# zjwzcx/GenNBV

Measured on AMD Instinct MI355X. Metric: env-steps/sec at 256 envs x 64^3 grid (state encoding + policy forward + GAE + PPO update), higher is better.
Workload: dtype f32

## Files before the change

gennbv_amd/csrc/conv_split.h:

```cpp
#pragma once
#include <type_traits>

typedef _Float16 h8 __attribute__((ext_vector_type(8)));
typedef _Float16 h4 __attribute__((ext_vector_type(4)));
typedef _Float16 h2 __attribute__((ext_vector_type(2)));

namespace split {
constexpr int kThreads = 1024, kWaves = 16;
constexpr int kConsWaves = 8, kProdThreads = 512;
constexpr int kNP = 4, kNPl = 2 * kNP + 1;
constexpr int kRing = 5;
constexpr int kRowBytes = 2048;
constexpr int kStageBytes = kNPl * kRing * kRowBytes;
constexpr int kPadBytes = 64;
constexpr int kSlots = (2 * kNPl * 128 + kProdThreads - 1) / kProdThreads;
constexpr int kRedBytes = 2 * kNP * 1024;
constexpr int kDyBytes = 2 * kNP * 1024;
constexpr int kGradBits = 14;
constexpr int kLdsBytes = kStageBytes + kPadBytes + kRedBytes;
constexpr int kWgLdsBytes = kStageBytes + kPadBytes + kDyBytes;
constexpr int kKSteps = 14, kKHalf = 7;
constexpr float kZScale = 256.0f, kWScale = 1024.0f, kZMax = 65000.0f;
constexpr int kW2ImgU4 = kKSteps * 2 * 64;

// ... 411 lines not shown
constexpr int kChunks = 5;
static_assert(4 * split::kNPl + split::kNP == kChunks * (split::kWaves - split::kConsWaves), "40 chunks over 8 staging waves");
}

__device__ __forceinline__ void glds16_nt(const void *gsrc, uint32_t lds_dst)
{
    uint32_t keep;
    asm volatile("s_mov_b32 %0, m0\n\ts_mov_b32 m0, %2\n\ts_nop 0\n\tglobal_load_lds_dwordx4 %1, off nt\n\ts_mov_b32 m0, %0"
                 : "=&s"(keep) : "v"(gsrc), "s"(lds_dst) : "memory");
}
template <int N>
__device__ __forceinline__ void wait_vm_keep()
{
    asm volatile("s_waitcnt vmcnt(%0)" ::"n"(N) : "memory");
}
__device__ __forceinline__ uint32_t lds_addr(const void *p)
{
    return (uint32_t)(uintptr_t)(__attribute__((address_space(3))) const char *)p;
}

__global__ __launch_bounds__(split::kThreads) void k_conv2_wgrad_split_dma(
    const float *__restrict__ y1, const float *__restrict__ scale1, const float *__restrict__ shift1, const float *__restrict__ dy2 ,
    const unsigned *__restrict__ absmax, int B, int O1, int O2, int nitems, float *__restrict__ partial )
{
    using namespace split;
    extern __shared__ __attribute__((aligned(16))) char split_lds[];
    char *stage = split_lds, *dyst = split_lds + wdma::kStageBytes + kPadBytes;
    constexpr int R = wdma::kRing;
    const int tid = threadIdx.x, lane = tid & (kWave - 1), wv = __builtin_amdgcn_readfirstlane(tid / kWave);
    constexpr int E2 = kTaps * 256 + kC;
    float *out = partial + (size_t)blockIdx.x * E2;
    if (tid < kPadBytes / 16) reinterpret_cast<uint4 *>(split_lds + wdma::kStageBytes)[tid] = make_uint4(0, 0, 0, 0);
    const int P2 = O2 * O2 * O2;
    const int nsteps = (O2 + 1) & ~1;
    if (wv >= kConsWaves) {
        const int pw = wv - kConsWaves, q = lane & 3, vx = lane >> 2;
        const bool dy_wave = pw >= 4;
        const uint32_t rowC = 2 * 16 * kC, planeC = rowC * (uint32_t)O1;
        const int dpl = pw - 4;
        const uint32_t stage_a = lds_addr(stage), dy_a = lds_addr(dyst);
        float gs = 1.0f, sc[4] = {0.f, 0.f, 0.f, 0.f}, sh[4] = {0.f, 0.f, 0.f, 0.f};
        bool first = true;
        for (int item = (int)blockIdx.x; item < nitems; item += (int)gridDim.x) {
            int b, oz0, oz1;
            if (!sample_plane_group(B, O2, kNP, b, oz0, oz1, item)) continue;
            const int np = oz1 - oz0, npl = 2 * np + 1;
            const float *ybase = y1 + ((size_t)b * O1 + 2 * oz0) * planeC + lane * 4;
            const bool dvalid = dy_wave && dpl < np && vx < O2;
            const float *dsrc = dy2 + ((size_t)b * P2 + (size_t)(oz0 + min(max(dpl, 0), np - 1)) * O2 * O2 + min(vx, O2 - 1)) * kC + 4 * q;
            auto issue = [&](int j) {
#ifdef WDMA_ABL_NODMA
                return;
#endif
#pragma unroll
                for (int k = 0; k < wdma::kChunks; ++k) {
                    if (k == wdma::kChunks - 1 && dy_wave) {
                        glds16_nt(dsrc + (size_t)min(max(j, 0), O2 - 1) * O2 * kC, __builtin_amdgcn_readfirstlane(dy_a + (uint32_t)((((j + 3) % wdma::kDyBufs) * kNP + dpl) * 1024)));
                    } else {
                        const int h = pw + 8 * k, pi = h >> 2, row = 2 * j + 1 + ((h >> 1) & 1), slot = (row + 2 * R) % R;
                        const float *src = ybase + (uint32_t)min(pi, npl - 1) * planeC + (uint32_t)min(max(row, 0), O1 - 1) * rowC + (h & 1) * (16 * kC);
                        glds16_nt(src, __builtin_amdgcn_readfirstlane(stage_a + (uint32_t)((pi * R + slot) * kRowBytes + (h & 1) * 1024)));
                    }
                }
            };
            auto convert = [&](int j) {
#ifdef WDMA_ABL_NOCONV
                return;
#endif
                char *cp[wdma::kChunks];
                float4 raw[wdma::kChunks];
#pragma unroll
                for (int k = 0; k < wdma::kChunks; ++k) {
                    if (k == wdma::kChunks - 1 && dy_wave) {
                        cp[k] = dyst + (((j + 3) % wdma::kDyBufs) * kNP + dpl) * 1024;
                    } else {
                        const int h = pw + 8 * k, pi = h >> 2, row = 2 * j + 1 + ((h >> 1) & 1), slot = (row + 2 * R) % R;
                        cp[k] = stage + (pi * R + slot) * kRowBytes + (h & 1) * 1024;
                    }
                    raw[k] = *reinterpret_cast<const float4 *>(cp[k] + lane * 16);
                }
#pragma unroll
                for (int k = 0; k < wdma::kChunks; ++k) {
                    float z[4];
                    const float v[4] = {raw[k].x, raw[k].y, raw[k].z, raw[k].w};
                    if (k == wdma::kChunks - 1 && dy_wave) {
#pragma unroll
                        for (int e = 0; e < 4; ++e) z[e] = dvalid ? v[e] * gs : 0.0f;
                    } else {
                        const bool pad_voxel = ((pw + 8 * k) & 1) == 1 && vx == 15;
#pragma unroll
                        for (int e = 0; e < 4; ++e) z[e] = pad_voxel ? 0.0f : __builtin_amdgcn_fmed3f(fmaf(sc[e], v[e], sh[e]), 0.f, kZMax);
                    }
                    h4 hi, lo;
#pragma unroll
                    for (int e = 0; e < 4; ++e) {
                        _Float16 a, c2;
                        split2(z[e], a, c2);
                        hi[e] = a;
                        lo[e] = c2;
                    }
                    char *dst = cp[k] + vx * 32 + q * 8;
                    *reinterpret_cast<h4 *>(dst) = hi;
#ifndef SPLIT_HI_ONLY
                    *reinterpret_cast<h4 *>(dst + 512) = lo;
#endif
                }
            };
            issue(-1);
            issue(0);
            if (first) {
                gs = grad_scale(absmax);
#pragma unroll
                for (int s = 0; s < 4; ++s) {
                    sc[s] = scale1[4 * q + s] * kZScale;
                    sh[s] = shift1[4 * q + s] * kZScale;
                }
                first = false;
            }
#pragma unroll
            for (int s = 0; s < 4; ++s) asm volatile("" : "+v"(sc[s]), "+v"(sh[s]));
            wait_vm_keep<0>();
            convert(-1);
            issue(1);
            convert(0);
            split_step_barrier();
            for (int t = 1; t <= nsteps; ++t) {
                issue(t + 1);
                wait_vm_keep<wdma::kChunks>();
                convert(t);
                split_step_barrier();
            }
            wait_vm_keep<0>();
        }
    } else {
        const float gs = grad_scale(absmax);
        const int n = lane & 15, g = lane >> 4, cw = wv;
        const int ntaps = cw < 3 ? 4 : 3;
        uint32_t tapbase[4];
        int tapdy[4];
#pragma unroll
        for (int i = 0; i < 4; ++i) {
            const int tp = min(cw + 8 * i, kTaps - 1), dz = tp / 9, dy = (tp / 3) % 3, dx = tp % 3;
            tapbase[i] = (uint32_t)(dz * R * kRowBytes + (dx == 1 ? 1024 : 0) + (dx == 2 ? 32 : 0)) + lane * 8;
            tapdy[i] = dy;
        }
        f32x4 acc[4];
#pragma unroll
        for (int i = 0; i < 4; ++i) acc[i] = (f32x4){0.f, 0.f, 0.f, 0.f};
        h8 ones;
#pragma unroll
        for (int e = 0; e < 8; ++e) ones[e] = (_Float16)1.0f;
        for (int item = (int)blockIdx.x; item < nitems; item += (int)gridDim.x) {
            int b, oz0, oz1;
            if (!sample_plane_group(B, O2, kNP, b, oz0, oz1, item)) continue;
            const int np = oz1 - oz0;
            split_step_barrier();
            for (int t = 1; t <= nsteps; ++t) {
                const int oy = t - 1;
#ifdef WDMA_ABL_NOCOMP
                if (false) {
#else
                if (oy < O2) {
#endif
                    uint32_t rowoff[3];
#pragma unroll
                    for (int dy = 0; dy < 3; ++dy) rowoff[dy] = (uint32_t)(((2 * oy + dy) % R) * kRowBytes);
                    const char *dybuf = dyst + (oy % wdma::kDyBufs) * kNP * 1024 + lane * 8;
#pragma unroll
                    for (int kb = 0; kb < 2; ++kb) {
                        if (2 * kb < np) {
                            const h8 bh = tr_pair(dybuf + (2 * kb) * 1024, dybuf + (2 * kb + 1) * 1024);
                            const h8 bl = tr_pair(dybuf + (2 * kb) * 1024 + 512, dybuf + (2 * kb + 1) * 1024 + 512);
                            h8 ah[4], al[4];
#pragma unroll
                            for (int i = 0; i < 4; ++i) {
                                if (i < 3 || ntaps == 4) {
                                    const uint32_t off = tapbase[i] + (tapdy[i] == 0 ? rowoff[0] : tapdy[i] == 1 ? rowoff[1] : rowoff[2]);
                                    const char *a0 = stage + (2 * (2 * kb)) * R * kRowBytes + off, *a1 = a0 + 2 * R * kRowBytes;
                                    ah[i] = tr_pair(a0, a1);
                                    al[i] = tr_pair(a0 + 512, a1 + 512);
                                }
                            }
#pragma unroll
                            for (int i = 0; i < 3; ++i) acc[i] = mfma_h(ah[i], bh, acc[i]);
                            if (ntaps == 4) acc[3] = mfma_h(ah[3], bh, acc[3]);
#pragma unroll
                            for (int i = 0; i < 3; ++i) acc[i] = mfma_lo(al[i], bh, acc[i]);
                            if (ntaps == 4) acc[3] = mfma_lo(al[3], bh, acc[3]);
#pragma unroll
                            for (int i = 0; i < 3; ++i) acc[i] = mfma_lo(ah[i], bl, acc[i]);
                            if (ntaps == 4) acc[3] = mfma_lo(ah[3], bl, acc[3]);
                            if (cw == 7) {
                                acc[3] = mfma_h(ones, bh, acc[3]);
                                acc[3] = mfma_lo(ones, bl, acc[3]);
                            }
                        }
                    }
                }
                split_step_barrier();
            }
// ... 465 lines not shown
    const float *__restrict__ dy2, const uint4 *__restrict__ w2img , const float *__restrict__ wbound ,
    const unsigned *__restrict__ absmax, const float *__restrict__ y1,
    const float *__restrict__ scale1, const float *__restrict__ shift1, const float *__restrict__ mean1, const float *__restrict__ rstd1,
    const int8_t *__restrict__ grid_i8, const int64_t *__restrict__ rows, int64_t grid_row_stride, int B, int G, int O1, int O2,
    float *__restrict__ partial )
{
    conv2_dgrad_c1w_split_body(dy2, w2img, wbound, absmax, y1, scale1, shift1, mean1, rstd1, grid_i8, rows, grid_row_stride, B, G, O1, O2, partial,
                               (int)blockIdx.x);
}


namespace fsplit {
constexpr int kInPlanes = 2 * split::kNPl + 1;
constexpr int kInRows = 5;
constexpr int kInRowBytes = 128, kInPlaneBytes = kInRows * kInRowBytes;
constexpr int kInBuf = kInPlanes * kInPlaneBytes + 64;
constexpr int kInPieces = kInPlanes * kInRows * 4;
constexpr int kTilesPerStep = 2 * split::kNPl * 2;
constexpr int kCompWaves = 4, kStageWaves = 12;
constexpr int kTilesPerWave = kTilesPerStep / kStageWaves;
static_assert(kTilesPerWave * kStageWaves == kTilesPerStep && kStageWaves % 4 == 0 && (kCompWaves + kStageWaves) * 64 == split::kThreads, "tile split");
constexpr float kW1Scale = 1024.0f;
constexpr int kLdsBytes = split::kStageBytes + split::kPadBytes + split::kRedBytes + 2 * kInBuf;
}

__global__ void k_prep_w2_split_only(const float *__restrict__ W2, float *__restrict__ w2img)
{
    prep_w2_split_items<true>(W2, w2img, blockIdx.x * blockDim.x + threadIdx.x, gridDim.x * blockDim.x);
}

template <bool TRAIN>
__global__ __launch_bounds__(split::kThreads) void k_conv12_fwd_split(
    const int8_t *__restrict__ grid_i8, const int64_t *__restrict__ rows, int64_t grid_row_stride, const float *__restrict__ W1 ,
    const float *__restrict__ b1, const float *__restrict__ scale1, const float *__restrict__ shift1, int B, int G, int O1, int O2,
    const uint4 *__restrict__ w2img, const float *__restrict__ b2, float *__restrict__ y2, float *__restrict__ y1 ,
    float *__restrict__ partials )
{
    using namespace split;
    using namespace fsplit;
    extern __shared__ __attribute__((aligned(16))) char split_lds[];
    char *stage = split_lds;
    float *red = reinterpret_cast<float *>(split_lds + split::kStageBytes + kPadBytes);
    char *inbuf = split_lds + split::kStageBytes + kPadBytes + kRedBytes;
    int b, oz0, oz1;
    const bool live = sample_plane_group(B, O2, kNP, b, oz0, oz1);
    const int tid = threadIdx.x, lane = tid & (kWave - 1), wv = __builtin_amdgcn_readfirstlane(tid / kWave);
    if (!live) {
        if (TRAIN) write_partials(partials, kWaves, wv, 0.f, 0.f);
        return;
    }
    const int np = oz1 - oz0;
    const int nsteps = (O2 + 2) & ~1;
    float s_sum = 0.0f, s_sq = 0.0f;
    if (wv >= kCompWaves) {
        const int ptid = tid - kCompWaves * kWave, pw = min(max(wv - kCompWaves, 0), kStageWaves - 1);
        const int n = lane & 15, g = lane >> 4;
        h8 wh, wl, wh2, wl2;
#pragma unroll
        for (int e = 0; e < 8; ++e) {
            const int r = 2 * g + (e >> 2), dx = e & 3;
            _Float16 hi, lo;
            split2(dx < 3 ? W1[n * kTaps + 3 * r + dx] * kW1Scale : 0.0f, hi, lo);
            wh[e] = hi;
            wl[e] = lo;
            split2(g == 0 && e < 3 ? W1[n * kTaps + 24 + e] * kW1Scale : 0.0f, hi, lo);
            wh2[e] = hi;
            wl2[e] = lo;
        }
        const int rsel = (pw >> 1) & 1, par = pw & 1;
        auto row_addr = [&](int r) {
            return (uint32_t)(split::kStageBytes + kPadBytes + kRedBytes + (r / 3 + 2 * (pw >> 2)) * kInPlaneBytes + (r % 3 + 2 * rsel) * kInRowBytes + 2 * (4 * n + 2 * par));
        };
        uint32_t tapaddr[3] = {row_addr(2 * g), row_addr(2 * g + 1), row_addr(8)};
        float bb[4], sc[4], sh[4];
#pragma unroll
        for (int r = 0; r < 4; ++r) {
            bb[r] = b1[4 * g + r];
            sc[r] = scale1[4 * g + r] * kZScale;
            sh[r] = shift1[4 * g + r] * kZScale;
            if (!TRAIN) {
                sh[r] = fmaf(sc[r], bb[r], sh[r]);
                sc[r] *= 1.0f / kW1Scale;
            }
        }
        const int f = min(ptid, kInPieces - 1), fpl = f / (kInRows * 4), frow = (f >> 2) % kInRows, fq = f & 3;
        const int8_t *in = grid_i8 + (rows ? rows[b] : (int64_t)b) * grid_row_stride;
        const int plane_g = min(4 * oz0 + fpl, G - 1);
        auto in_req = [&](int j) {
            const int row_g = min(max(4 * j + 2 + frow, 0), G - 1);
            const int8_t *src = in + ((size_t)plane_g * G + row_g) * G + 16 * fq;
            if constexpr (TRAIN) {
                u4v_t v;
                ldu4_nt_async(v, src);
                return v;
            } else {
                const uint4 u = ldu4_nt(src);
                return (u4v_t){u.x, u.y, u.z, u.w};
            }
        };
        auto in_store = [&](int j, const u4v_t &v) {
            const uint32_t w[4] = {v[0] ^ 0x80808080u, v[1] ^ 0x80808080u, v[2] ^ 0x80808080u, v[3] ^ 0x80808080u};
            uint32_t o[8];
#pragma unroll
            for (int q = 0; q < 4; ++q) {
                const h2 bias = {(_Float16)1152.0f, (_Float16)1152.0f};
                const uint32_t p0 = __builtin_amdgcn_perm(0x64646464u, w[q], 0x04010400u), p1 = __builtin_amdgcn_perm(0x64646464u, w[q], 0x04030402u);
                const h2 f0 = *reinterpret_cast<const h2 *>(&p0) - bias, f1 = *reinterpret_cast<const h2 *>(&p1) - bias;
                o[2 * q] = *reinterpret_cast<const uint32_t *>(&f0);
                o[2 * q + 1] = *reinterpret_cast<const uint32_t *>(&f1);
            }
            if (ptid < kInPieces) {
                uint4 *dst = reinterpret_cast<uint4 *>(inbuf + (j & 1) * kInBuf + fpl * kInPlaneBytes + frow * kInRowBytes + 32 * fq);
                dst[0] = make_uint4(o[0], o[1], o[2], o[3]);
                dst[1] = make_uint4(o[4], o[5], o[6], o[7]);
            }
        };
        if (ptid < 8) reinterpret_cast<uint4 *>(inbuf + (ptid >> 2) * kInBuf + kInPlanes * kInPlaneBytes)[ptid & 3] = make_uint4(0, 0, 0, 0);
        const uint32_t y1_lane = (uint32_t)((par * 16 + n) * kC + 4 * g), y1_pad = (uint32_t)((16 + 15) * kC + 4 * g);
        auto compute = [&](int j, const int jp ) {
            auto gather = [&](int k, h8 &xa, h8 &xc) {
                uint32_t d[6];
#pragma unroll
                for (int r = 0; r < 3; ++r) {
                    const uint32_t *src = reinterpret_cast<const uint32_t *>(split_lds + tapaddr[r] + (uint32_t)(jp * kInBuf + 6 * k * kInPlaneBytes));
                    d[2 * r] = src[0];
                    d[2 * r + 1] = src[1];
                }
                const uint4 ua = make_uint4(d[0], d[1], d[2], d[3]), uc = make_uint4(d[4], d[5], d[4], d[5]);
                xa = *reinterpret_cast<const h8 *>(&ua);
                xc = *reinterpret_cast<const h8 *>(&uc);
            };
            const int row = 2 * j + 1 + rsel, slot = (row + kRing) % kRing;
#pragma unroll
            for (int e = 0; e < 3; ++e) asm volatile("" : "+v"(tapaddr[e]));
            h8 xb, xb2;
            gather(0, xb, xb2);
#pragma unroll
            for (int k = 0; k < kTilesPerWave; ++k) {
                const int pi = (pw >> 2) + 3 * k;
                f32x4 acc = {0.f, 0.f, 0.f, 0.f};
                acc = mfma_h(wh, xb, acc);
                acc = mfma_h(wh2, xb2, acc);
                acc = mfma_lo(wl, xb, acc);
                acc = mfma_lo(wl2, xb2, acc);
                if (k + 1 < kTilesPerWave) gather(k + 1, xb, xb2);
                h4 hi, lo;
                float yv[4];
#pragma unroll
                for (int r = 0; r < 4; ++r) {
                    const float y = TRAIN ? acc[r] * (1.0f / kW1Scale) + bb[r] : acc[r];
                    yv[r] = y;
                    _Float16 a, c2;
                    split2(__builtin_amdgcn_fmed3f(fmaf(sc[r], y, sh[r]), 0.f, kZMax), a, c2);
                    hi[r] = a;
                    lo[r] = c2;
                }
                if (TRAIN) {
                    const int own = __builtin_amdgcn_readfirstlane((int)(row >= 0) & (int)(row < O1) & ((int)(pi < 2 * np) | ((int)(pi == 2 * np) & (int)(oz1 == O2))));
                    const uint32_t rowbase = vox1(b, min(2 * oz0 + pi, O1 - 1), min(max(row, 0), O1 - 1), 0, O1) * kC;
                    char *dst1 = reinterpret_cast<char *>(y1 + __builtin_amdgcn_readfirstlane(rowbase));
#ifdef FSPLIT_ABL_NOSTORE
                    st4_nt_masked(dst1, 4 * y1_pad, (f32x4){yv[0], yv[1], yv[2], yv[3]}, 1u, 0u);
#else
                    st4_nt_masked(dst1, own ? 4 * y1_lane : 4 * y1_pad, (f32x4){yv[0], yv[1], yv[2], yv[3]}, own ? ~0u : 1u, own ? ~0u : 0u);
#endif
                }
                char *dst = stage + (pi * kRing + slot) * kRowBytes + par * 1024 + n * 32 + g * 8;
                *reinterpret_cast<h4 *>(dst) = hi;
#ifndef SPLIT_HI_ONLY
                *reinterpret_cast<h4 *>(dst + 512) = lo;
#endif
            }
        };
        constexpr int kVmHalf = kTilesPerWave + 1, kVmFull = 2 * kTilesPerWave + 1;
        static_assert(kTilesPerWave == 3 && kVmHalf == 4 && kVmFull == 7, "the explicit vmcnt waits of the training forward's staging waves assume "
                      "kTilesPerWave y1 stores + one input request per half step (re-derive them when kNPl / kStageWaves change)");
        u4v_t ra = in_req(-1), rb = in_req(0);
        if constexpr (TRAIN) wait_vm_keep1<1>(ra);
        in_store(-1, ra);
        ra = in_req(1);
        split_step_barrier();
        compute(-1, 1);
        if constexpr (TRAIN) wait_vm_keep1<kVmHalf>(rb);
        in_store(0, rb);
        rb = in_req(2);
        split_step_barrier();
        compute(0, 0);
        if constexpr (TRAIN) wait_vm_keep1<kVmFull>(ra);
        in_store(1, ra);
        ra = in_req(3);
        split_step_barrier();
        for (int t = 1; t <= nsteps; t += 2) {
            compute(t, 1);
            if constexpr (TRAIN) wait_vm_keep1<kVmFull>(rb);
            in_store(t + 1, rb);
            rb = in_req(t + 3);
            split_step_barrier();
            compute(t + 1, 0);
            if constexpr (TRAIN) wait_vm_keep1<kVmFull>(ra);
            in_store(t + 2, ra);
            ra = in_req(t + 4);
            split_step_barrier();
        }
    } else {
        const int m = lane & 15, g = lane >> 4;
        const int pl2 = wv >> 1, kh = wv & 1;
        h8 wh[kKHalf], wl[kKHalf];
#pragma unroll
        for (int s = 0; s < kKHalf; ++s) {
            const uint4 uh = w2img[((kh * kKHalf + s) * 2 + 0) * 64 + lane], ul = w2img[((kh * kKHalf + s) * 2 + 1) * 64 + lane];
            wh[s] = *reinterpret_cast<const h8 *>(&uh);
            wl[s] = *reinterpret_cast<const h8 *>(&ul);
        }
        const float bias = b2[m];
        const int P2 = O2 * O2 * O2;
        const bool second = (g >> 1) != 0;
        f32x4 prev0 = {0.f, 0.f, 0.f, 0.f}, prev1 = prev0;
        auto plane_step = [&](const int q, f32x4 &prev, int t) {
            const int oy = t - 1, pl = 2 * pl2 + q;
            const uint32_t a_lane = (uint32_t)(2 * pl * kRing * kRowBytes + m * 32 + (g & 1) * 16);
            if (kh == 0 && pl < np && oy >= 1 && oy - 1 < O2) {
                const f32x4 other = *reinterpret_cast<const f32x4 *>(red + (((t - 1) & 1) * kNP + pl) * 256 + lane * 4);
                const f32x4 acc = (prev + other) * (1.0f / (kZScale * kWScale));
                float *out = y2 + ((size_t)b * kC + m) * P2 + (size_t)(oz0 + pl) * O2 * O2 + (size_t)(oy - 1) * O2;
#pragma unroll
                for (int rr = 0; rr < 4; ++rr) {
                    const int oxi = 4 * g + rr;
                    if (oxi < O2) {
                        const float y = acc[rr] + bias;
                        out[oxi] = y;
                        if (TRAIN) {
                            s_sum += y;
                            s_sq += y * y;
                        }
                    }
                }
            }
            if (pl < np && oy < O2) {
                uint32_t rowoff[3];
#pragma unroll
                for (int dy = 0; dy < 3; ++dy) rowoff[dy] = (uint32_t)(((2 * oy + dy) % kRing) * kRowBytes);
                auto tap_off = [&](int tp) {
                    const int dz = tp / 9, dy = (tp / 3) % 3, dx = tp % 3;
                    return (uint32_t)(dz * kRing * kRowBytes + (dx == 1 ? 1024 : 0) + (dx == 2 ? 32 : 0)) + rowoff[dy];
                };
                auto a_off = [&](int s) {
                    const uint32_t ta = kh ? tap_off(2 * (kKHalf + s)) : tap_off(2 * s);
                    const uint32_t tb = kh ? tap_off(min(2 * (kKHalf + s) + 1, kTaps - 1)) : tap_off(2 * s + 1);
                    return a_lane + (second ? tb : ta);
                };
                f32x4 acc_hh = {0.f, 0.f, 0.f, 0.f}, acc_lh = acc_hh, acc_hl = acc_hh;
                constexpr int kAhead = 2;
                h8 ah[kAhead + 1], al[kAhead + 1];
#pragma unroll
                for (int s = 0; s < kAhead; ++s) {
                    ah[s] = *reinterpret_cast<const h8 *>(stage + a_off(s));
                    al[s] = *reinterpret_cast<const h8 *>(stage + a_off(s) + 512);
                }
#pragma unroll
                for (int s = 0; s < kKHalf; ++s) {
                    if (s + kAhead < kKHalf) {
                        ah[(s + kAhead) % (kAhead + 1)] = *reinterpret_cast<const h8 *>(stage + a_off(s + kAhead));
                        al[(s + kAhead) % (kAhead + 1)] = *reinterpret_cast<const h8 *>(stage + a_off(s + kAhead) + 512);
                    }
                    acc_hh = mfma_h(ah[s % (kAhead + 1)], wh[s], acc_hh);
                    acc_lh = mfma_lo(al[s % (kAhead + 1)], wh[s], acc_lh);
                    acc_hl = mfma_lo(ah[s % (kAhead + 1)], wl[s], acc_hl);
                    __builtin_amdgcn_sched_barrier(0);
                }
                const f32x4 part = acc_hh + (acc_lh + acc_hl);
                if (kh)
                    *reinterpret_cast<f32x4 *>(red + ((t & 1) * kNP + pl) * 256 + lane * 4) = part;
                else
                    prev = part;
            }
        };
        split_step_barrier();
        split_step_barrier();
        split_step_barrier();
        for (int t = 1; t <= nsteps; ++t) {
            plane_step(0, prev0, t);
            plane_step(1, prev1, t);
            split_step_barrier();
        }
    }
    if (TRAIN) write_partials(partials, kWaves, wv, s_sum, s_sq);
}


__global__ __launch_bounds__(kEncThreads) void k_conv1_fwd_split(
    const int8_t *__restrict__ grid_i8, const int64_t *__restrict__ rows, int64_t grid_row_stride, int B, int G, int O1, const float *__restrict__ W1,
    const float *__restrict__ b1, float *__restrict__ y1, const float *__restrict__ W2, float *__restrict__ w2img)
{
    using namespace split;
    prep_w2_in_passing(W2, w2img);
    __shared__ __attribute__((aligned(16))) int8_t s_in[3 * 64 * 64 + 64];
    int b, oz;
    if (!sample_plane(B, O1, b, oz)) return;
    const int tid = threadIdx.x, lane = tid & (kWave - 1), wv = __builtin_amdgcn_readfirstlane(tid / kWave);
    const int n = lane & 15, g = lane >> 4;
    const int8_t *in = grid_i8 + (rows ? rows[b] : (int64_t)b) * grid_row_stride + (size_t)(2 * oz) * G * G;
    {
        uint4 v[3];
#pragma unroll
        for (int u = 0; u < 3; ++u) v[u] = *reinterpret_cast<const uint4 *>(in + 16 * (u * kEncThreads + tid));
#pragma unroll
        for (int u = 0; u < 3; ++u) reinterpret_cast<uint4 *>(s_in)[u * kEncThreads + tid] = v[u];
        if (tid < 4) reinterpret_cast<uint4 *>(s_in)[768 + tid] = make_uint4(0, 0, 0, 0);
    }
    h8 wh, wl;
#pragma unroll
    for (int e = 0; e < 8; ++e) {
        const int t = 8 * g + e;
        _Float16 hi, lo;
        split2(t < kTaps ? W1[n * kTaps + t] * fsplit::kW1Scale : 0.0f, hi, lo);
        wh[e] = hi;
        wl[e] = lo;
    }
    uint32_t tapoff[8];
// ... 25 lines not shown
```

gennbv_amd/csrc/encoder.hip:

```cpp
#include <cstdlib>

#include "common.h"
#include "../../include/gennbv_hip.h"

typedef float f32x4 __attribute__((ext_vector_type(4)));
constexpr int kC = 16;
constexpr int kTaps = 27;
constexpr int kEncThreads = 256;
constexpr int kEncWaves = kEncThreads / kWave;

__device__ __forceinline__ uint32_t vox1(int b, int z, int y, int x, int O1)
{
    const uint32_t XH = (uint32_t)(O1 + 1) >> 1;
    return ((((uint32_t)b * O1 + z) * O1 + y) * 2 + (x & 1)) * XH + ((uint32_t)x >> 1);
}
static inline size_t y1_elems(int batch, int O1) { return (size_t)batch * O1 * O1 * 2 * ((O1 + 1) / 2) * kC; }

struct ActF32 {
    typedef float T;
    static __device__ __forceinline__ float4 ld4(const T *p) { return *reinterpret_cast<const float4 *>(p); }
    static __device__ __forceinline__ void st4(T *p, float4 v) { *reinterpret_cast<float4 *>(p) = v; }
    static __device__ __forceinline__ float ld1(const T *p) { return *p; }
};

// ... 1750 lines not shown
    const int O1 = out_size(grid), O2 = out_size(O1);
    return eval_prepare_launches(p, batch, O1, O2 * O2 * O2, bn_state, enc_carve(workspace, batch, grid), gnbv_stream(stream), true);
}

GNBV_API int gnbv_encoder_grid_forward(const float *obs_grid, const int64_t *rows, int64_t row_stride, int batch, int grid,
                                       const GnbvEncoderParams *p, int training, const int *skip_flag, void *y1, float *y2,
                                       float *bn_state , float *features,
                                       void *workspace, size_t workspace_bytes, void *stream)
{
    GNBV_CHECK_ARG(p && (obs_grid || (p->grid_i8)) && y1 && y2 && bn_state && workspace && batch > 0 && grid >= 7);
    GNBV_CHECK_ARG(p->grid_i8 == nullptr || p->grid_i8_row_stride >= (int64_t)grid * grid * grid);
    GNBV_CHECK_ARG(workspace_bytes >= gnbv_encoder_workspace_bytes(batch, grid) && ((uintptr_t)workspace & 255) == 0);
    GNBV_CHECK_ARG(p->w1 && p->b1 && p->bn1_w && p->bn1_b && p->bn1_rm && p->bn1_rv && p->w2 && p->b2 && p->bn2_w && p->bn2_b &&
                   p->bn2_rm && p->bn2_rv);
    hipStream_t st = gnbv_stream(stream);
    const int O1 = out_size(grid), O2 = out_size(O1);
    GNBV_CHECK_ARG(O2 >= 1 && y1_elems(batch, O1) < ((size_t)1 << 31));
    const int P2 = O2 * O2 * O2;
    EncWs w = enc_carve(workspace, batch, grid);
    float *bn1 = bn_state, *bn2 = bn_state + 4 * kC;
    int err;
    GNBV_CHECK_ARG(p->autocorr == nullptr || (p->autocorr_row_stride >= kAcRow && p->autocorr_row_stride % 4 == 0 && ((uintptr_t)p->autocorr & 15) == 0));
    const bool dp = training && p->world > 1 && p->sync_sum != nullptr && p->sync_buf != nullptr;
    const bool fused_eval = !training && conv_split_path(p, grid) && conv1_i8_staged(p, grid) && grid == 64 && !env_off("GENNBV_FUSED_EVAL");
    bool fused_train = false;
    if (fused_eval) {
        if (!p->eval_prepared && (err = eval_prepare_launches(p, batch, O1, P2, bn_state, w, st, false))) return err;
        static bool attr_fe = false;
        if (!attr_fe) {
            const hipError_t e = hipFuncSetAttribute((const void *)k_conv12_fwd_split<false>, hipFuncAttributeMaxDynamicSharedMemorySize, fsplit::kLdsBytes);
            if (e != hipSuccess) return (int)e;
            attr_fe = true;
        }
        hipLaunchKernelGGL(k_conv12_fwd_split<false>, dim3(sample_plane_group_grid(batch, O2, split::kNP)), dim3(split::kThreads), fsplit::kLdsBytes, st,
                           p->grid_i8, rows, p->grid_i8_row_stride, p->w1, p->b1, (const float *)bn1, (const float *)(bn1 + kC), batch, grid, O1, O2,
                           (const uint4 *)w.w2split, p->b2, y2, (float *)nullptr, (float *)nullptr);
        if ((err = gnbv_launch_status())) return err;
    } else {
    const bool analytic = training && analytic_bn1(p, grid);
    if (dp && !(analytic && fused_path(p, grid) && p->autocorr_global != nullptr)) return (int)hipErrorInvalidValue;
    fused_train = analytic && conv_split_path(p, grid) && grid == 64 && !env_off("GENNBV_CONV1_SPLIT") && !env_off("GENNBV_FUSED_TRAIN");
    if (analytic) {
        const bool have_total = p->autocorr_total != nullptr && !dp;
        hipLaunchKernelGGL(k_bn1_analytic, dim3(fused_train ? 9 : 1), dim3(1024), 0, st, have_total ? (const int *)p->autocorr_total : (const int *)p->autocorr,
                           p->autocorr_row_stride, rows, have_total ? 0 : batch, p->w1,
                           p->b1, p->bn1_w, p->bn1_b, p->eps, p->momentum, p->bn1_rm, p->bn1_rv, p->bn1_nbt, skip_flag, bn1, bn1 + kC, bn1 + 2 * kC,
                           bn1 + 3 * kC, (int *)(bn_state + kBnStateFloats), dp ? (const int *)p->autocorr_global : (const int *)nullptr,
                           p->w2, w.w2img, p->range_flag);
        if ((err = gnbv_launch_status())) return err;
    }
    float *c1_part = (training && !analytic) ? w.bn_part : nullptr;
    const int split_img = (conv_split_path(p, grid) || conv_splitx_path(p, grid)) ? 1 : 0;
    if (fused_train) {
        static bool attr_ft = false;
        if (!attr_ft) {
            const hipError_t e = hipFuncSetAttribute((const void *)k_conv12_fwd_split<true>, hipFuncAttributeMaxDynamicSharedMemorySize, fsplit::kLdsBytes);
            if (e != hipSuccess) return (int)e;
            attr_ft = true;
        }
        hipLaunchKernelGGL(k_conv12_fwd_split<true>, dim3(sample_plane_group_grid(batch, O2, split::kNP)), dim3(split::kThreads), fsplit::kLdsBytes, st,
                           p->grid_i8, rows, p->grid_i8_row_stride, p->w1, p->b1, (const float *)bn1, (const float *)(bn1 + kC), batch, grid, O1, O2,
                           (const uint4 *)w.w2split, p->b2, y2, (float *)y1, w.bn_part);
    } else {
        const size_t c1_lds = (size_t)3 * (2 * O1 + 1) * grid * sizeof(float);
        const bool c1_staged = obs_grid != nullptr && (grid % 4 == 0) && (row_stride % 4 == 0) && (((uintptr_t)obs_grid & 15) == 0) && c1_lds <= 64 * 1024 &&
                               2 * O1 + 1 <= grid;
        if (conv1_i8_staged(p, grid) && c1_part == nullptr && grid == 64 && conv_split_path(p, grid) && !env_off("GENNBV_CONV1_SPLIT"))
            hipLaunchKernelGGL(k_conv1_fwd_split, dim3(sample_plane_grid(batch, O1)), dim3(kEncThreads), 0, st, p->grid_i8, rows, p->grid_i8_row_stride, batch, grid,
                               O1, p->w1, p->b1, (float *)y1, p->w2, w.w2img);
        else if (conv1_i8_staged(p, grid))
            hipLaunchKernelGGL((k_conv1_fwd_lds<ActF32, int8_t>), dim3(sample_plane_grid(batch, O1)), dim3(kEncThreads), c1_lds, st, p->grid_i8, rows,
                               p->grid_i8_row_stride, batch, grid, O1, p->w1, p->b1, (float *)y1, c1_part, p->w2, w.w2img, split_img);
        else if (c1_staged)
            hipLaunchKernelGGL((k_conv1_fwd_lds<ActF32, float>), dim3(sample_plane_grid(batch, O1)), dim3(kEncThreads), c1_lds, st, obs_grid, rows,
                               row_stride, batch, grid, O1, p->w1, p->b1, (float *)y1, c1_part, p->w2, w.w2img, split_img);
        else if (p->grid_i8 != nullptr && grid % 16 == 0 && p->grid_i8_row_stride % 16 == 0 && (((uintptr_t)p->grid_i8 & 15) == 0) &&
                 c1_lds / 4 <= 64 * 1024 && 2 * O1 + 1 <= grid)
            hipLaunchKernelGGL((k_conv1_fwd_lds<ActF32, int8_t, true>), dim3(sample_plane_grid(batch, O1)), dim3(kEncThreads), c1_lds / 4, st, p->grid_i8,
                               rows, p->grid_i8_row_stride, batch, grid, O1, p->w1, p->b1, (float *)y1, c1_part, p->w2, w.w2img, split_img);
        else if (obs_grid == nullptr)
            hipLaunchKernelGGL((k_conv1_fwd<ActF32, int8_t>), dim3(sample_plane_grid(batch, O1)), dim3(kEncThreads), 0, st, p->grid_i8, rows,
                               p->grid_i8_row_stride, batch, grid, O1, p->w1, p->b1, (float *)y1, c1_part, p->w2, w.w2img, split_img);
        else
            hipLaunchKernelGGL(k_conv1_fwd<ActF32>, dim3(sample_plane_grid(batch, O1)), dim3(kEncThreads), 0, st, obs_grid, rows, row_stride,
                               batch, grid, O1, p->w1, p->b1, (float *)y1, c1_part, p->w2, w.w2img, split_img);
    }
    if ((err = gnbv_launch_status())) return err;
    if (analytic) {
    } else if (training)
        hipLaunchKernelGGL(k_stats_reduce, dim3(1), dim3(1024), 0, st, w.bn_part, sample_plane_grid(batch, O1), (double *)nullptr,
                           (double)batch * O1 * O1 * O1, p->bn1_w, p->bn1_b, p->eps, p->momentum, p->bn1_rm, p->bn1_rv, p->bn1_nbt, skip_flag,
                           bn1, bn1 + kC, bn1 + 2 * kC, bn1 + 3 * kC, (const float *)nullptr, (float *)nullptr, p->w1, p->b1, p->range_flag);
    else
        hipLaunchKernelGGL(k_bn_finalize, dim3(1), dim3(64), 0, st, (double)batch * O1 * O1 * O1, p->bn1_w, p->bn1_b, p->eps, p->momentum,
// ... 279 lines not shown
```

Baseline: 49030.

## Make split conv kernels persistent with cross-item prefetch of next work item

Converts the fused conv1+conv2 forward kernel into a persistent kernel with a grid capped at the max resident workgroups, looping over work items. Both it and the wgrad DMA kernel now prefetch the next item's input rows during the tail steps of the current item, using a global ring index so the staging slots stay consistent across items. This removes the pipeline drain and refill and the per-block launch overhead between items. Per-item BN partials are now written per item through a small LDS reduction. The cost is more complex indexing and serialized work per block, which can hurt load balance.

Result: faster. 50650, median of 6 (+3.3%).

```diff
diff --git a/gennbv_amd/csrc/conv_split.h b/gennbv_amd/csrc/conv_split.h
--- a/gennbv_amd/csrc/conv_split.h
+++ b/gennbv_amd/csrc/conv_split.h
@@ -467,7 +467,7 @@
     float *out = partial + (size_t)blockIdx.x * E2;
     if (tid < kPadBytes / 16) reinterpret_cast<uint4 *>(split_lds + wdma::kStageBytes)[tid] = make_uint4(0, 0, 0, 0);
     const int P2 = O2 * O2 * O2;
-    const int nsteps = (O2 + 1) & ~1;
+    const int S = O2 + 1;
     if (wv >= kConsWaves) {
         const int pw = wv - kConsWaves, q = lane & 3, vx = lane >> 2;
         const bool dy_wave = pw >= 4;
@@ -475,95 +475,111 @@
         const int dpl = pw - 4;
         const uint32_t stage_a = lds_addr(stage), dy_a = lds_addr(dyst);
         float gs = 1.0f, sc[4] = {0.f, 0.f, 0.f, 0.f}, sh[4] = {0.f, 0.f, 0.f, 0.f};
-        bool first = true;
-        for (int item = (int)blockIdx.x; item < nitems; item += (int)gridDim.x) {
+        struct Item {
+            const float *ybase, *dbase;
+            int np, j0;
+        };
+        const uint32_t ylane = lane * 4, dlane = (uint32_t)(min(vx, O2 - 1) * kC + 4 * q);
+        auto take = [&](Item &it, int item, int j0) {
             int b, oz0, oz1;
-            if (!sample_plane_group(B, O2, kNP, b, oz0, oz1, item)) continue;
-            const int np = oz1 - oz0, npl = 2 * np + 1;
-            const float *ybase = y1 + ((size_t)b * O1 + 2 * oz0) * planeC + lane * 4;
+            if (item >= nitems || !sample_plane_group(B, O2, kNP, b, oz0, oz1, item)) return false;
+            it.np = oz1 - oz0, it.j0 = j0;
+            it.ybase = y1 + ((size_t)b * O1 + 2 * oz0) * planeC;
+            it.dbase = dy2 + ((size_t)b * P2 + (size_t)(oz0 + min(max(dpl, 0), it.np - 1)) * O2 * O2) * kC;
+            return true;
+        };
+        auto issue = [&](const Item &it, int J) {
+#ifdef WDMA_ABL_NODMA
+            return;
+#endif
+            const int j = J - it.j0, npl = 2 * it.np + 1;
+#pragma unroll
+            for (int k = 0; k < wdma::kChunks; ++k) {
+                if (k == wdma::kChunks - 1 && dy_wave) {
+                    glds16_nt(it.dbase + dlane + (size_t)min(max(j, 0), O2 - 1) * O2 * kC, __builtin_amdgcn_readfirstlane(dy_a + (uint32_t)((((J + 3) % wdma::kDyBufs) * kNP + dpl) * 1024)));
+                } else {
+                    const int h = pw + 8 * k, pi = h >> 2, rpar = (h >> 1) & 1, row = 2 * j + 1 + rpar, slot = (2 * J + 1 + rpar + 2 * R) % R;
+                    const float *src = it.ybase + ylane + (uint32_t)min(pi, npl - 1) * planeC + (uint32_t)min(max(row, 0), O1 - 1) * rowC + (h & 1) * (16 * kC);
+                    glds16_nt(src, __builtin_amdgcn_readfirstlane(stage_a + (uint32_t)((pi * R + slot) * kRowBytes + (h & 1) * 1024)));
+                }
+            }
+        };
+        auto convert = [&](int np, int J) {
+#ifdef WDMA_ABL_NOCONV
+            return;
+#endif
             const bool dvalid = dy_wave && dpl < np && vx < O2;
-            const float *dsrc = dy2 + ((size_t)b * P2 + (size_t)(oz0 + min(max(dpl, 0), np - 1)) * O2 * O2 + min(vx, O2 - 1)) * kC + 4 * q;
-            auto issue = [&](int j) {
-#ifdef WDMA_ABL_NODMA
-                return;
+            char *cp[wdma::kChunks];
+            float4 raw[wdma::kChunks];
+#pragma unroll
+            for (int k = 0; k < wdma::kChunks; ++k) {
+                if (k == wdma::kChunks - 1 && dy_wave) {
+                    cp[k] = dyst + (((J + 3) % wdma::kDyBufs) * kNP + dpl) * 1024;
+                } else {
+                    const int h = pw + 8 * k, pi = h >> 2, slot = (2 * J + 1 + ((h >> 1) & 1) + 2 * R) % R;
+                    cp[k] = stage + (pi * R + slot) * kRowBytes + (h & 1) * 1024;
+                }
+                raw[k] = *reinterpret_cast<const float4 *>(cp[k] + lane * 16);
+            }
+            asm volatile("" ::: "memory");
+#pragma unroll
+            for (int k = 0; k < wdma::kChunks; ++k) {
+                float z[4];
+                const float v[4] = {raw[k].x, raw[k].y, raw[k].z, raw[k].w};
+                if (k == wdma::kChunks - 1 && dy_wave) {
+#pragma unroll
+                    for (int e = 0; e < 4; ++e) z[e] = dvalid ? v[e] * gs : 0.0f;
+                } else {
+                    const bool pad_voxel = ((pw + 8 * k) & 1) == 1 && vx == 15;
+#pragma unroll
+                    for (int e = 0; e < 4; ++e) z[e] = pad_voxel ? 0.0f : __builtin_amdgcn_fmed3f(fmaf(sc[e], v[e], sh[e]), 0.f, kZMax);
+                }
+                h4 hi, lo;
+#pragma unroll
+                for (int e = 0; e < 4; ++e) {
+                    _Float16 a, c2;
+                    split2(z[e], a, c2);
+                    hi[e] = a;
+                    lo[e] = c2;
+                }
+                char *dst = cp[k] + vx * 32 + q * 8;
+                *reinterpret_cast<h4 *>(dst) = hi;
+#ifndef SPLIT_HI_ONLY
+                *reinterpret_cast<h4 *>(dst + 512) = lo;
 #endif
-#pragma unroll
-                for (int k = 0; k < wdma::kChunks; ++k) {
-                    if (k == wdma::kChunks - 1 && dy_wave) {
-                        glds16_nt(dsrc + (size_t)min(max(j, 0), O2 - 1) * O2 * kC, __builtin_amdgcn_readfirstlane(dy_a + (uint32_t)((((j + 3) % wdma::kDyBufs) * kNP + dpl) * 1024)));
-                    } else {
-                        const int h = pw + 8 * k, pi = h >> 2, row = 2 * j + 1 + ((h >> 1) & 1), slot = (row + 2 * R) % R;
-                        const float *src = ybase + (uint32_t)min(pi, npl - 1) * planeC + (uint32_t)min(max(row, 0), O1 - 1) * rowC + (h & 1) * (16 * kC);
-                        glds16_nt(src, __builtin_amdgcn_readfirstlane(stage_a + (uint32_t)((pi * R + slot) * kRowBytes + (h & 1) * 1024)));
-                    }
-                }
-            };
-            auto convert = [&](int j) {
-#ifdef WDMA_ABL_NOCONV
-                return;
-#endif
-                char *cp[wdma::kChunks];
-                float4 raw[wdma::kChunks];
-#pragma unroll
-                for (int k = 0; k < wdma::kChunks; ++k) {
-                    if (k == wdma::kChunks - 1 && dy_wave) {
-                        cp[k] = dyst + (((j + 3) % wdma::kDyBufs) * kNP + dpl) * 1024;
-                    } else {
-                        const int h = pw + 8 * k, pi = h >> 2, row = 2 * j + 1 + ((h >> 1) & 1), slot = (row + 2 * R) % R;
-                        cp[k] = stage + (pi * R + slot) * kRowBytes + (h & 1) * 1024;
-                    }
-                    raw[k] = *reinterpret_cast<const float4 *>(cp[k] + lane * 16);
-                }
-#pragma unroll
-                for (int k = 0; k < wdma::kChunks; ++k) {
-                    float z[4];
-                    const float v[4] = {raw[k].x, raw[k].y, raw[k].z, raw[k].w};
-                    if (k == wdma::kChunks - 1 && dy_wave) {
-#pragma unroll
-                        for (int e = 0; e < 4; ++e) z[e] = dvalid ? v[e] * gs : 0.0f;
-                    } else {
-                        const bool pad_voxel = ((pw + 8 * k) & 1) == 1 && vx == 15;
-#pragma unroll
-                        for (int e = 0; e < 4; ++e) z[e] = pad_voxel ? 0.0f : __builtin_amdgcn_fmed3f(fmaf(sc[e], v[e], sh[e]), 0.f, kZMax);
-                    }
-                    h4 hi, lo;
-#pragma unroll
-                    for (int e = 0; e < 4; ++e) {
-                        _Float16 a, c2;
-                        split2(z[e], a, c2);
-                        hi[e] = a;
-                        lo[e] = c2;
-                    }
-                    char *dst = cp[k] + vx * 32 + q * 8;
-                    *reinterpret_cast<h4 *>(dst) = hi;
-#ifndef SPLIT_HI_ONLY
-                    *reinterpret_cast<h4 *>(dst + 512) = lo;
-#endif
-                }
-            };
-            issue(-1);
-            issue(0);
-            if (first) {
-                gs = grad_scale(absmax);
-#pragma unroll
-                for (int s = 0; s < 4; ++s) {
-                    sc[s] = scale1[4 * q + s] * kZScale;
-                    sh[s] = shift1[4 * q + s] * kZScale;
-                }
-                first = false;
+            }
+        };
+        Item cur;
+        if (take(cur, (int)blockIdx.x, 0)) {
+            issue(cur, -1);
+            issue(cur, 0);
+            gs = grad_scale(absmax);
+#pragma unroll
+            for (int s = 0; s < 4; ++s) {
+                sc[s] = scale1[4 * q + s] * kZScale;
+                sh[s] = shift1[4 * q + s] * kZScale;
             }
 #pragma unroll
             for (int s = 0; s < 4; ++s) asm volatile("" : "+v"(sc[s]), "+v"(sh[s]));
             wait_vm_keep<0>();
-            convert(-1);
-            issue(1);
-            convert(0);
+            convert(cur.np, -1);
+            issue(cur, 1);
+            convert(cur.np, 0);
             split_step_barrier();
-            for (int t = 1; t <= nsteps; ++t) {
-                issue(t + 1);
-                wait_vm_keep<wdma::kChunks>();
-                convert(t);
-                split_step_barrier();
+            for (int item = (int)blockIdx.x;;) {
+                Item nxt = cur;
+                const bool more = take(nxt, item + (int)gridDim.x, cur.j0 + S);
+                for (int tt = 1; tt <= S; ++tt) {
+                    const int T = cur.j0 + tt;
+                    const bool in = tt >= S - 2, cn = tt >= S - 1;
+                    const Item is = {in ? nxt.ybase : cur.ybase, in ? nxt.dbase : cur.dbase, in ? nxt.np : cur.np, in ? nxt.j0 : cur.j0};
+                    issue(is, T + 1);
+                    wait_vm_keep<wdma::kChunks>();
+                    convert(cn ? nxt.np : cur.np, T);
+                    split_step_barrier();
+                }
+                if (!more) break;
+                cur = nxt, item += (int)gridDim.x;
             }
             wait_vm_keep<0>();
         }
@@ -585,13 +601,14 @@
         h8 ones;
 #pragma unroll
         for (int e = 0; e < 8; ++e) ones[e] = (_Float16)1.0f;
-        for (int item = (int)blockIdx.x; item < nitems; item += (int)gridDim.x) {
-            int b, oz0, oz1;
-            if (!sample_plane_group(B, O2, kNP, b, oz0, oz1, item)) continue;
-            const int np = oz1 - oz0;
-            split_step_barrier();
-            for (int t = 1; t <= nsteps; ++t) {
-                const int oy = t - 1;
+        int b, oz0, oz1, j0 = 0;
+        bool more = (int)blockIdx.x < nitems && sample_plane_group(B, O2, kNP, b, oz0, oz1, (int)blockIdx.x);
+        if (more) split_step_barrier();
+        for (int item = (int)blockIdx.x; more; item += (int)gridDim.x, j0 += S) {
+            const int np = __builtin_amdgcn_readfirstlane(oz1 - oz0);
+            more = item + (int)gridDim.x < nitems && sample_plane_group(B, O2, kNP, b, oz0, oz1, item + (int)gridDim.x);
+            for (int tt = 1; tt <= S; ++tt) {
+                const int oy = tt - 1, roy = j0 + oy;
 #ifdef WDMA_ABL_NOCOMP
                 if (false) {
 #else
@@ -599,8 +616,8 @@
 #endif
                     uint32_t rowoff[3];
 #pragma unroll
-                    for (int dy = 0; dy < 3; ++dy) rowoff[dy] = (uint32_t)(((2 * oy + dy) % R) * kRowBytes);
-                    const char *dybuf = dyst + (oy % wdma::kDyBufs) * kNP * 1024 + lane * 8;
+                    for (int dy = 0; dy < 3; ++dy) rowoff[dy] = (uint32_t)(((2 * roy + dy) % R) * kRowBytes);
+                    const char *dybuf = dyst + (roy % wdma::kDyBufs) * kNP * 1024 + lane * 8;
 #pragma unroll
                     for (int kb = 0; kb < 2; ++kb) {
                         if (2 * kb < np) {
@@ -1132,26 +1149,37 @@
 template <bool TRAIN>
 __global__ __launch_bounds__(split::kThreads) void k_conv12_fwd_split(
     const int8_t *__restrict__ grid_i8, const int64_t *__restrict__ rows, int64_t grid_row_stride, const float *__restrict__ W1 ,
-    const float *__restrict__ b1, const float *__restrict__ scale1, const float *__restrict__ shift1, int B, int G, int O1, int O2,
+    const float *__restrict__ b1, const float *__restrict__ scale1, const float *__restrict__ shift1, int B, int G, int O1, int O2, int nitems,
     const uint4 *__restrict__ w2img, const float *__restrict__ b2, float *__restrict__ y2, float *__restrict__ y1 ,
     float *__restrict__ partials )
 {
     using namespace split;
     using namespace fsplit;
     extern __shared__ __attribute__((aligned(16))) char split_lds[];
+    __shared__ float bn2x[2][2 * kC];
     char *stage = split_lds;
     float *red = reinterpret_cast<float *>(split_lds + split::kStageBytes + kPadBytes);
     char *inbuf = split_lds + split::kStageBytes + kPadBytes + kRedBytes;
-    int b, oz0, oz1;
-    const bool live = sample_plane_group(B, O2, kNP, b, oz0, oz1);
     const int tid = threadIdx.x, lane = tid & (kWave - 1), wv = __builtin_amdgcn_readfirstlane(tid / kWave);
-    if (!live) {
-        if (TRAIN) write_partials(partials, kWaves, wv, 0.f, 0.f);
+    const int nsteps = (O2 + 2) & ~1;
+    const int stride = (int)gridDim.x;
+    struct Item {
+        const int8_t *in;
+        int b, oz0, np, top, j0;
+    };
+    auto take = [&](Item &it, int item, int j0) {
+        int b, oz0, oz1;
+        if (item >= nitems || !sample_plane_group(B, O2, kNP, b, oz0, oz1, item)) return false;
+        it.b = b, it.oz0 = oz0, it.np = oz1 - oz0, it.top = (int)(oz1 == O2), it.j0 = j0;
+        it.in = grid_i8 + (rows ? rows[b] : (int64_t)b) * grid_row_stride;
+        return true;
+    };
+    Item cur;
+    if (!take(cur, (int)blockIdx.x, 0)) {
+        if (TRAIN && tid < 2 * kC)
+            for (int item = (int)blockIdx.x; item < nitems; item += stride) partials[(size_t)item * 2 * kC + tid] = 0.0f;
         return;
     }
-    const int np = oz1 - oz0;
-    const int nsteps = (O2 + 2) & ~1;
-    float s_sum = 0.0f, s_sq = 0.0f;
     if (wv >= kCompWaves) {
         const int ptid = tid - kCompWaves * kWave, pw = min(max(wv - kCompWaves, 0), kStageWaves - 1);
         const int n = lane & 15, g = lane >> 4;
@@ -1184,11 +1212,10 @@
             }
         }
         const int f = min(ptid, kInPieces - 1), fpl = f / (kInRows * 4), frow = (f >> 2) % kInRows, fq = f & 3;
-        const int8_t *in = grid_i8 + (rows ? rows[b] : (int64_t)b) * grid_row_stride;
-        const int plane_g = min(4 * oz0 + fpl, G - 1);
-        auto in_req = [&](int j) {
+        auto in_req = [&](const int8_t *in, int oz0, int j0, int J) {
+            const int j = J - j0, plane_g = min(4 * oz0 + fpl, G - 1);
             const int row_g = min(max(4 * j + 2 + frow, 0), G - 1);
-            const int8_t *src = in + ((size_t)plane_g * G + row_g) * G + 16 * fq;
+            const int8_t *src = in + (uint32_t)((plane_g * G + row_g) * G + 16 * fq);
             if constexpr (TRAIN) {
                 u4v_t v;
                 ldu4_nt_async(v, src);
@@ -1217,7 +1244,7 @@
         };
         if (ptid < 8) reinterpret_cast<uint4 *>(inbuf + (ptid >> 2) * kInBuf + kInPlanes * kInPlaneBytes)[ptid & 3] = make_uint4(0, 0, 0, 0);
         const uint32_t y1_lane = (uint32_t)((par * 16 + n) * kC + 4 * g), y1_pad = (uint32_t)((16 + 15) * kC + 4 * g);
-        auto compute = [&](int j, const int jp ) {
+        auto compute = [&](const Item &it, int J, const int jp ) {
             auto gather = [&](int k, h8 &xa, h8 &xc) {
                 uint32_t d[6];
 #pragma unroll
@@ -1230,7 +1257,7 @@
                 xa = *reinterpret_cast<const h8 *>(&ua);
                 xc = *reinterpret_cast<const h8 *>(&uc);
             };
-            const int row = 2 * j + 1 + rsel, slot = (row + kRing) % kRing;
+            const int row = 2 * (J - it.j0) + 1 + rsel, slot = (2 * J + 1 + rsel + kRing) % kRing;
 #pragma unroll
             for (int e = 0; e < 3; ++e) asm volatile("" : "+v"(tapaddr[e]));
             h8 xb, xb2;
@@ -1256,8 +1283,8 @@
                     lo[r] = c2;
                 }
                 if (TRAIN) {
-                    const int own = __builtin_amdgcn_readfirstlane((int)(row >= 0) & (int)(row < O1) & ((int)(pi < 2 * np) | ((int)(pi == 2 * np) & (int)(oz1 == O2))));
-                    const uint32_t rowbase = vox1(b, min(2 * oz0 + pi, O1 - 1), min(max(row, 0), O1 - 1), 0, O1) * kC;
+                    const int own = __builtin_amdgcn_readfirstlane((int)(row >= 0) & (int)(row < O1) & ((int)(pi < 2 * it.np) | ((int)(pi == 2 * it.np) & it.top)));
+                    const uint32_t rowbase = vox1(it.b, min(2 * it.oz0 + pi, O1 - 1), min(max(row, 0), O1 - 1), 0, O1) * kC;
                     char *dst1 = reinterpret_cast<char *>(y1 + __builtin_amdgcn_readfirstlane(rowbase));
 #ifdef FSPLIT_ABL_NOSTORE
                     st4_nt_masked(dst1, 4 * y1_pad, (f32x4){yv[0], yv[1], yv[2], yv[3]}, 1u, 0u);
@@ -1275,32 +1302,41 @@
         constexpr int kVmHalf = kTilesPerWave + 1, kVmFull = 2 * kTilesPerWave + 1;
         static_assert(kTilesPerWave == 3 && kVmHalf == 4 && kVmFull == 7, "the explicit vmcnt waits of the training forward's staging waves assume "
                       "kTilesPerWave y1 stores + one input request per half step (re-derive them when kNPl / kStageWaves change)");
-        u4v_t ra = in_req(-1), rb = in_req(0);
+        u4v_t ra = in_req(cur.in, cur.oz0, 0, -1), rb = in_req(cur.in, cur.oz0, 0, 0);
         if constexpr (TRAIN) wait_vm_keep1<1>(ra);
         in_store(-1, ra);
-        ra = in_req(1);
+        ra = in_req(cur.in, cur.oz0, 0, 1);
         split_step_barrier();
-        compute(-1, 1);
+        compute(cur, -1, 1);
         if constexpr (TRAIN) wait_vm_keep1<kVmHalf>(rb);
         in_store(0, rb);
-        rb = in_req(2);
+        rb = in_req(cur.in, cur.oz0, 0, 2);
         split_step_barrier();
-        compute(0, 0);
+        compute(cur, 0, 0);
         if constexpr (TRAIN) wait_vm_keep1<kVmFull>(ra);
         in_store(1, ra);
-        ra = in_req(3);
+        ra = in_req(cur.in, cur.oz0, 0, 3);
         split_step_barrier();
-        for (int t = 1; t <= nsteps; t += 2) {
-            compute(t, 1);
-            if constexpr (TRAIN) wait_vm_keep1<kVmFull>(rb);
-            in_store(t + 1, rb);
-            rb = in_req(t + 3);
-            split_step_barrier();
-            compute(t + 1, 0);
-            if constexpr (TRAIN) wait_vm_keep1<kVmFull>(ra);
-            in_store(t + 2, ra);
-            ra = in_req(t + 4);
-            split_step_barrier();
+        for (int item = (int)blockIdx.x;;) {
+            Item nxt = cur;
+            const bool more = take(nxt, item + stride, cur.j0 + nsteps);
+            for (int tt = 1; tt <= nsteps; tt += 2) {
+                const int T = cur.j0 + tt;
+                const bool cn = tt >= nsteps - 1, rbn = tt + 3 >= nsteps - 1, ran = tt + 4 >= nsteps - 1;
+                const Item ci = {nullptr, cn ? nxt.b : cur.b, cn ? nxt.oz0 : cur.oz0, cn ? nxt.np : cur.np, cn ? nxt.top : cur.top, cn ? nxt.j0 : cur.j0};
+                compute(ci, T, 1);
+                if constexpr (TRAIN) wait_vm_keep1<kVmFull>(rb);
+                in_store(T + 1, rb);
+                rb = in_req(rbn ? nxt.in : cur.in, rbn ? nxt.oz0 : cur.oz0, rbn ? nxt.j0 : cur.j0, T + 3);
+                split_step_barrier();
+                compute(ci, T + 1, 0);
+                if constexpr (TRAIN) wait_vm_keep1<kVmFull>(ra);
+                in_store(T + 2, ra);
+                ra = in_req(ran ? nxt.in : cur.in, ran ? nxt.oz0 : cur.oz0, ran ? nxt.j0 : cur.j0, T + 4);
+                split_step_barrier();
+            }
+            if (!more) break;
+            cur = nxt, item += stride;
         }
     } else {
         const int m = lane & 15, g = lane >> 4;
@@ -1316,6 +1352,8 @@
         const int P2 = O2 * O2 * O2;
         const bool second = (g >> 1) != 0;
         f32x4 prev0 = {0.f, 0.f, 0.f, 0.f}, prev1 = prev0;
+        float s_sum = 0.0f, s_sq = 0.0f;
+        int b = cur.b, oz0 = cur.oz0, np = cur.np, j0 = 0;
         auto plane_step = [&](const int q, f32x4 &prev, int t) {
             const int oy = t - 1, pl = 2 * pl2 + q;
             const uint32_t a_lane = (uint32_t)(2 * pl * kRing * kRowBytes + m * 32 + (g & 1) * 16);
@@ -1339,7 +1377,7 @@
             if (pl < np && oy < O2) {
                 uint32_t rowoff[3];
 #pragma unroll
-                for (int dy = 0; dy < 3; ++dy) rowoff[dy] = (uint32_t)(((2 * oy + dy) % kRing) * kRowBytes);
+                for (int dy = 0; dy < 3; ++dy) rowoff[dy] = (uint32_t)(((2 * (j0 + oy) + dy) % kRing) * kRowBytes);
                 auto tap_off = [&](int tp) {
                     const int dz = tp / 9, dy = (tp / 3) % 3, dx = tp % 3;
                     return (uint32_t)(dz * kRing * kRowBytes + (dx == 1 ? 1024 : 0) + (dx == 2 ? 32 : 0)) + rowoff[dy];
@@ -1378,13 +1416,31 @@
         split_step_barrier();
         split_step_barrier();
         split_step_barrier();
-        for (int t = 1; t <= nsteps; ++t) {
-            plane_step(0, prev0, t);
-            plane_step(1, prev1, t);
-            split_step_barrier();
-        }
-    }
-    if (TRAIN) write_partials(partials, kWaves, wv, s_sum, s_sq);
+        for (int item = (int)blockIdx.x;;) {
+            for (int t = 1; t <= nsteps; ++t) {
+                plane_step(0, prev0, t);
+                plane_step(1, prev1, t);
+                if (TRAIN && t == nsteps) {
+                    const float s = kgroup_sum(s_sum), sq = kgroup_sum(s_sq);
+                    if (kh == 0 && lane < kC) {
+                        bn2x[pl2][lane] = s;
+                        bn2x[pl2][kC + lane] = sq;
+                    }
+                    s_sum = 0.0f, s_sq = 0.0f;
+                }
+                split_step_barrier();
+            }
+            if (TRAIN && wv == 0 && lane < 2 * kC) partials[(size_t)item * 2 * kC + lane] = bn2x[0][lane] + bn2x[1][lane];
+            item += stride;
+            int oz1;
+            if (item >= nitems || !sample_plane_group(B, O2, kNP, b, oz0, oz1, item)) {
+                if (TRAIN && wv == 0 && lane < 2 * kC)
+                    for (; item < nitems; item += stride) partials[(size_t)item * 2 * kC + lane] = 0.0f;
+                break;
+            }
+            np = oz1 - oz0, j0 += nsteps;
+        }
+    }
 }
 
 
diff --git a/gennbv_amd/csrc/encoder.hip b/gennbv_amd/csrc/encoder.hip
--- a/gennbv_amd/csrc/encoder.hip
+++ b/gennbv_amd/csrc/encoder.hip
@@ -1806,8 +1806,9 @@
             if (e != hipSuccess) return (int)e;
             attr_fe = true;
         }
-        hipLaunchKernelGGL(k_conv12_fwd_split<false>, dim3(sample_plane_group_grid(batch, O2, split::kNP)), dim3(split::kThreads), fsplit::kLdsBytes, st,
-                           p->grid_i8, rows, p->grid_i8_row_stride, p->w1, p->b1, (const float *)bn1, (const float *)(bn1 + kC), batch, grid, O1, O2,
+        const int nitems = sample_plane_group_grid(batch, O2, split::kNP);
+        hipLaunchKernelGGL(k_conv12_fwd_split<false>, dim3(min(nitems, conv_max_wg())), dim3(split::kThreads), fsplit::kLdsBytes, st,
+                           p->grid_i8, rows, p->grid_i8_row_stride, p->w1, p->b1, (const float *)bn1, (const float *)(bn1 + kC), batch, grid, O1, O2, nitems,
                            (const uint4 *)w.w2split, p->b2, y2, (float *)nullptr, (float *)nullptr);
         if ((err = gnbv_launch_status())) return err;
     } else {
@@ -1832,8 +1833,9 @@
             if (e != hipSuccess) return (int)e;
             attr_ft = true;
         }
-        hipLaunchKernelGGL(k_conv12_fwd_split<true>, dim3(sample_plane_group_grid(batch, O2, split::kNP)), dim3(split::kThreads), fsplit::kLdsBytes, st,
-                           p->grid_i8, rows, p->grid_i8_row_stride, p->w1, p->b1, (const float *)bn1, (const float *)(bn1 + kC), batch, grid, O1, O2,
+        const int nitems = sample_plane_group_grid(batch, O2, split::kNP);
+        hipLaunchKernelGGL(k_conv12_fwd_split<true>, dim3(min(nitems, conv_max_wg())), dim3(split::kThreads), fsplit::kLdsBytes, st,
+                           p->grid_i8, rows, p->grid_i8_row_stride, p->w1, p->b1, (const float *)bn1, (const float *)(bn1 + kC), batch, grid, O1, O2, nitems,
                            (const uint4 *)w.w2split, p->b2, y2, (float *)y1, w.bn_part);
     } else {
         const size_t c1_lds = (size_t)3 * (2 * O1 + 1) * grid * sizeof(float);
```
